# volume-em/empanada

Hardware: AMD Instinct MI355X
Metric: Mvox/s end-to-end 3D panoptic inference (incl. consensus); PQ vs CPU ref (higher is better)
Workload: dtype f32

## Files before the change

empanada_amd/_hip.py:

```python
import ctypes
import os

import torch

_HERE = os.path.dirname(os.path.abspath(__file__))
LIB_PATH = os.path.join(_HERE, 'libemp_hip.so')

MAX_KS = 11
MAX_CLASSES = 16
MAX_CENTERS = 4096


class HipError(RuntimeError):
    pass


_c = ctypes
_P = _c.c_void_p
_I = _c.c_int
_L = _c.c_int64
_F = _c.c_float
_U32 = _c.c_uint32

SIGNATURES = {
    'emp_version': (_I, []),
    'emp_last_error': (_c.c_char_p, []),
    'emp_device_count': (_I, []),
    'emp_bn_act_nhwc': (_I, [_P, _P, _P, _P, _I, _L, _I, _P, _L, _P]),
    'emp_dwconv_nhwc': (_I, [_P, _P, _P, _I, _I, _I, _I, _I, _P, _P]),
    'emp_upsample_bilinear': (_I, [_P, _I, _I, _I, _I, _P, _P, _I, _I, _P, _P]),
    'emp_conv_bn_act_proj_nhwc': (_I, [_P, _P, _P, _P, _I] + [_I] * 10 + [_P, _I, _P, _P, _L, _P]),
    'emp_conv_k_slab': (_I, [_L, _I, _I, _I]),
    'emp_conv_k_slab_cin': (_I, [_L, _I, _I, _I, _I]),
    'emp_conv_k_slab_geom': (_I, [_L, _I, _I, _I, _I, _I, _I, _I, _I]),
    'emp_conv1x1_ws_eligible': (_I, [_L, _I, _I, _I, _I, _I, _I, _I]),
    'emp_gconv_chunk': (_I, [_I]),
    'emp_gconv3x3_bn_act_nhwc': (_I, [_P, _L, _P, _P, _P, _I, _I, _I, _I, _I, _I, _I, _P, _L, _P]),
    'emp_conv_bn_act_nhwc': (_I, [_P, _P, _P, _P, _P, _L, _I] + [_I] * 10 + [_P, _L, _P]),
    'emp_conv_splitk_plan': (_I, [_L, _I, _I, _I, _I]),
    'emp_conv_splitk_bn_act_nhwc': (_I, [_P, _P, _P, _P, _P, _L, _I] + [_I] * 11 + [_P, _P, _L, _P]),
    'emp_wino_input_transform': (_I, [_P, _I, _I, _I, _I, _I, _P, _L, _P, _P]),
    'emp_gemm_nt_batched': (_I, [_P, _P, _I, _L, _I, _I, _P, _P]),
    'emp_wino4_input_transform': (_I, [_P, _I, _I, _I, _I, _I, _P, _L, _P, _P]),
    'emp_wino4_output_transform': (_I, [_P, _P, _L, _I, _I, _I, _I, _I, _P, _P, _I, _P, _L, _P]),
    'emp_wino3_input_transform': (_I, [_P, _I, _I, _I, _I, _I, _P, _L, _P, _P]),
    'emp_wino3_output_transform': (_I, [_P, _P, _L, _I, _I, _I, _I, _I, _P, _P, _I, _P, _L, _P]),
    'emp_wino_gemm_fused': (_I, [_P, _I, _I, _I, _I, _I, _P, _L, _P, _I, _P, _P]),
    'emp_wino_output_transform': (_I, [_P, _P, _L, _I, _I, _I, _I, _I, _P, _P, _I, _P, _L, _P]),
    'emp_chain_class': (_I, [_L, _P, _P, _P, _I, _P, _P, _P, _P, _L, _L, _c.c_double, _c.c_double, _P, _P, _P, _P]),
    'emp_lsap_maximize': (_L, [_P, _L, _L, _P, _P]),
    'emp_slices_to_input': (_I, [_P, _L, _L, _L, _I, _I, _I, _I, _I, _F, _F, _P, _P]),
    'emp_pointwise_out_nhwc': (_I, [_P, _P, _P, _L, _L, _I, _I, _P, _P]),
    'emp_bn_relu_maxpool_nhwc': (_I, [_P, _P, _P, _I, _I, _I, _I, _P, _P]),
    'emp_stem_conv7_bn_relu_maxpool': (_I, [_P, _P, _P, _P, _I, _I, _I, _P, _P]),
    'emp_logits_to_prob': (_I, [_P, _I, _I, _L, _P, _P]),
    'emp_pr_upsample2x': (_I, [_P, _I, _I, _I, _I, _P, _P, _P]),
    'emp_pr_topk_work_bytes': (_L, [_I, _L]),
    'emp_pr_topk': (_I, [_P, _I, _L, _I, _P, _L, _P, _P]),
    'emp_pr_point_sample': (_I, [_P, _L, _P, _I, _I, _I, _I, _I, _P, _I, _I, _I, _P, _P, _I, _P]),
    'emp_pr_scatter': (_I, [_P, _I, _P, _I, _I, _I, _L, _P, _P]),
    'emp_median_harden_stack': (_I, [_P, _I, _I, _L, _I, _F, _P, _P, _P]),
    'emp_median_step': (_I, [_c.POINTER(_P), _I, _L, _P, _P]),
    'emp_harden': (_I, [_P, _I, _I, _L, _F, _P, _P]),
    'emp_find_centers': (_I, [_P, _I, _I, _I, _F, _I, _I, _P, _P, _P]),
    'emp_group_work_elems': (_L, [_I, _I]),
    'emp_group_pixels': (_I, [_P, _P, _I, _P, _I, _I, _I, _I, _P, _U32, _P, _P, _P]),
    'emp_fuse_work_elems': (_L, [_I, _I, _I]),
    'emp_fuse_panoptic': (_I, [_P, _P, _I, _I, _I, _I, _I, _I, _U32, _L, _L, _L, _P, _P, _P, _P]),
    'emp_fuse_lut': (_I, [_P, _P, _I, _I, _I, _I, _I, _I, _U32, _L, _L, _P, _P]),
    'emp_fuse_apply': (_I, [_P, _P, _I, _I, _I, _I, _I, _I, _U32, _L, _L, _P, _P, _P, _P]),
    'emp_runs_count': (_I, [_P, _I, _I, _I, _P, _P]),
    'emp_scan_tmp_elems': (_L, [_L]),
    'emp_exclusive_scan_i32': (_I, [_P, _L, _P, _P, _P]),
    'emp_runs_extract': (_I, [_P, _I, _I, _I, _P, _P, _P, _P, _P]),
    'emp_runs_label_work_elems': (_L, [_L]),
    'emp_runs_label': (_I, [_P, _P, _P, _P, _L, _I, _I, _I, _L, _U32, _P, _P, _P, _P, _P, _P, _P, _P, _P]),
    'emp_runs_overlap_next': (_I, [_P, _P, _P, _P, _P, _L, _I, _I, _I, _L, _P, _L, _P, _P]),
    'emp_rle_decode': (_I, [_P, _P, _P, _L, _P, _P]),
    'emp_rle_encode_work_elems': (_L, [_L]),
    'emp_rle_encode': (_I, [_P, _L, _P, _P, _P, _P, _P]),
    'emp_box_pairs': (_I, [_P, _L, _P, _L, _I, _P, _P, _I, _P, _L, _P, _P]),
    'emp_rle_pair_intersections': (_I, [_P, _P, _P, _P, _L, _P, _P]),
    'emp_sort_work_bytes': (_L, [_L]),
    'emp_sort_u64_i32': (_I, [_P, _P, _P, _P, _L, _I, _I, _P, _L, _P]),
# ... 30 lines not shown
            fn = getattr(lib, name)
            fn.restype = res
            fn.argtypes = args
        _lib = lib
    return _lib


def require_gpu():
    if torch.cuda._is_in_bad_fork():
        raise HipError("this process was forked from one that had initialised the GPU: HIP cannot be used here.  Start "
                       "the process with the 'spawn' method (multiprocessing.set_start_method('spawn')), or call "
                       "patterns.forward_matching / forward_multigpu, which re-start themselves that way")
    if not torch.cuda.is_available():
        raise HipError("empanada_amd needs an MI355X (HIP device) for this operation; no CPU fallback exists")


def _ptr(t):
    if t is None:
        return None
    assert t.is_cuda and t.is_contiguous(), "device-resident contiguous tensor required"
    return t.data_ptr()


def as_u32(t):
    if t.dtype == torch.uint32:
        return t
    if t.dtype != torch.int32:
        t = t.to(torch.int32)
    return t.contiguous().view(torch.uint32)


def np_to_dev_u32(a):
    import numpy as np
    a = np.ascontiguousarray(a).astype(np.uint32)
    return torch.from_numpy(a.view(np.int32)).cuda().view(torch.uint32)


def stream():
    return torch.cuda.current_stream().cuda_stream


PROFILE = None
PROFILE_SKIP = set()
_TRACE = None
if os.environ.get('EMP_TRACE_CALLS'):
    _TRACE = open(os.environ['EMP_TRACE_CALLS'], 'a', buffering=1)


def trace(msg):
    if _TRACE is not None:
        _TRACE.write('# ' + msg + '\n')


def call(name, *args, alg_bytes=None, alg_flops=None):
    lib = load()
    if _TRACE is not None:
        _TRACE.write(name + ' ' + ' '.join(str(a) for a in args if isinstance(a, (int, float)) and abs(a) < (1 << 40))
                     + '\n')
    if PROFILE is not None and name not in PROFILE_SKIP:
        e0 = torch.cuda.Event(enable_timing=True)
        e1 = torch.cuda.Event(enable_timing=True)
        e0.record()
        rc = getattr(lib, name)(*args)
        e1.record()
        PROFILE.setdefault(name, []).append((e0, e1, alg_bytes, alg_flops))
    else:
        rc = getattr(lib, name)(*args)
    if rc != 0:
        raise HipError(f"{name} failed ({rc}): {lib.emp_last_error().decode()}")


def query(name, *args):
    return getattr(load(), name)(*args)


def median_harden_stack(prob, ks, thr, want_prob=False):
    require_gpu()
    D, C, H, W = prob.shape
    prob = prob.contiguous()
    sem = torch.empty((D, H, W), dtype=torch.uint8, device=prob.device)
    outp = torch.empty_like(prob) if want_prob else None
    call('emp_median_harden_stack', _ptr(prob), D, C, H * W, int(ks), float(thr), _ptr(sem), _ptr(outp), stream())
    return (sem, outp) if want_prob else sem


def _expect(what, t, dtype=None, shape=None, numel=None):
    if not isinstance(t, torch.Tensor) or not t.is_cuda:
        raise HipError(f"{what}: expected a tensor on the GPU")
    if dtype is not None and t.dtype not in (dtype if isinstance(dtype, tuple) else (dtype,)):
        raise HipError(f"{what}: dtype {t.dtype}, expected {dtype}")
    if shape is not None and tuple(t.shape) != tuple(shape):
        raise HipError(f"{what}: shape {tuple(t.shape)}, expected {tuple(shape)}")
    if numel is not None and t.numel() != numel:
        raise HipError(f"{what}: {t.numel()} elements, expected {numel}")
    return t


def median_step(slices, out=None):
    require_gpu()
    ks = len(slices)
    if not 1 <= ks <= MAX_KS:
        raise HipError(f"median over {ks} slices (1..{MAX_KS} supported)")
    for i, s in enumerate(slices):
        _expect(f"median_step: slice {i}", s, torch.float32, slices[0].shape)
    slices = [s.contiguous() for s in slices]
    n = slices[0].numel()
    if out is None:
        out = torch.empty_like(slices[0])
    _expect("median_step: out", out, torch.float32, numel=n)
    arr = (_P * ks)(*[s.data_ptr() for s in slices])
    call('emp_median_step', arr, ks, n, _ptr(out), stream())
    return out


def find_centers(hmp, thr, k, cap=1024):
    require_gpu()
    _expect("find_centers: heat map", hmp, torch.float32)
    D, h, w = hmp.shape
# ... 649 lines not shown
    g = w_oihw.detach().double().cpu()

    def comb(a, b, c):
        return [(G[0] * a + G[1] * b) + G[2] * c for G in _WINO3_G]

    rows = comb(g[:, :, 0, :], g[:, :, 1, :], g[:, :, 2, :])
    U = []
    for r in rows:
        U.extend(comb(r[:, :, 0], r[:, :, 1], r[:, :, 2]))
    return torch.stack(U, dim=0).float().contiguous()


def wino3_conv_bn_act(x, U, tiles_dev, dil, scale=None, shift=None, relu=False, out=None):
    require_gpu()
    N, Cin, H, W = x.shape
    Cout = U.shape[1]
    assert x.is_cuda and x.dtype == torch.float32 and x.is_contiguous(memory_format=torch.channels_last)
    T = tiles_dev.shape[0]
    V = torch.empty((25, T, Cin), dtype=torch.float32, device=x.device)
    Mw = torch.empty((25, T, Cout), dtype=torch.float32, device=x.device)
    if out is None:
        out = torch.empty((N, Cout, H, W), dtype=torch.float32, device=x.device, memory_format=torch.channels_last)
    assert out.shape == (N, Cout, H, W) and out.stride(1) == 1
    ops = out.stride(3)
    assert out.stride(2) == W * ops and out.stride(0) == H * W * ops, "NHWC channel slice required"
    st = stream()
    call('emp_wino3_input_transform', x.data_ptr(), N, H, W, Cin, dil, _ptr(tiles_dev), T, _ptr(V), st,
         alg_bytes=4 * (x.numel() + V.numel()))
    call('emp_gemm_nt_batched', _ptr(V), _ptr(U), 25, T, Cout, Cin, _ptr(Mw), st,
         alg_bytes=4 * (V.numel() + U.numel() + Mw.numel()), alg_flops=2 * 25 * T * Cout * Cin)
    call('emp_wino3_output_transform', _ptr(Mw), _ptr(tiles_dev), T, N, H, W, Cout, dil, _ptr(scale), _ptr(shift),
         int(bool(relu)), out.data_ptr(), ops, st, alg_bytes=4 * (Mw.numel() + N * Cout * H * W))
    return out


def conv_bn_act_proj_nhwc(x, w_okkc, scale, shift, relu, proj_w, proj_b=None, stride=1, pad=0, dil=1, keep=False):
    require_gpu()
    N, Cin, H, W = x.shape
    Cout, KH, KW, _ = w_okkc.shape
    n = proj_w.shape[0]
    assert x.is_cuda and x.dtype == torch.float32 and x.is_contiguous(memory_format=torch.channels_last)
    OH = (H + 2 * pad - dil * (KH - 1) - 1) // stride + 1
    OW = (W + 2 * pad - dil * (KW - 1) - 1) // stride + 1
    acc = torch.zeros((N, n, OH, OW), dtype=torch.float32, device=x.device)
    act = (torch.empty((N, Cout, OH, OW), dtype=torch.float32, device=x.device, memory_format=torch.channels_last)
           if keep else None)
    call('emp_conv_bn_act_proj_nhwc', x.data_ptr(), _ptr(w_okkc), _ptr(scale), _ptr(shift), int(bool(relu)), N, H, W,
         Cin, Cout, KH, KW, stride, pad, dil, _ptr(proj_w), n, _ptr(acc), act.data_ptr() if keep else None, 0,
         stream(), alg_bytes=4 * (x.numel() + w_okkc.numel() + acc.numel() + (act.numel() if keep else 0)),
         alg_flops=2 * N * OH * OW * Cout * (Cin * KH * KW + n))
    if proj_b is not None:
        acc += proj_b.view(1, -1, 1, 1)
    return (acc, act) if keep else acc
```

empanada_amd/csrc/emp_conv.hip:

```cpp
#include "emp_common.h"
#include <stdlib.h>

typedef float f32x16 __attribute__((ext_vector_type(16)));

#define CG_BM 128
#define CG_BK 32
#define CG_THREADS 256

struct ConvGeom {
    const float *x, *w, *scale, *shift, *res;
    float *out;
    int N, H, W, Cin, OH, OW, Cout, KH, KW, stride, pad, dil, relu;
    int64_t M, out_ps, res_ps;
    int tiles_m, tiles_n;
    int64_t x_bs, w_bs, out_bs;
    const int32_t *tiles;
    const float *proj_w;
    float *proj_out;
    int proj_n;
    int64_t hw;
};

__device__ __attribute__((aligned(16))) float cg_zero_page[64];

// ... 645 lines not shown
    const int T = g.tiles_m * g.tiles_n;
    const dim3 grid(8 * ((T + 7) / 8), 1, k_splits);
    hipStream_t st = emp_stream(stream);
    if (pl.narrow)
        hipLaunchKernelGGL((conv_igemm_f32_kernel<1, 0, false, 32, false, true>), grid, dim3(CG_THREADS), 0, st, g);
    else
        hipLaunchKernelGGL((conv_igemm_f32_kernel<2, 0, false, 32, false, true>), grid, dim3(CG_THREADS), 0, st, g);
    EMP_CHECK_LAUNCH("emp_conv_splitk_bn_act_nhwc(partials)");
    const int64_t total = g.M * (Cout / 4);
    hipLaunchKernelGGL(splitk_reduce_kernel, dim3(emp_grid(total, 256, 4096)), dim3(256), 0, st, work, k_splits, g.M, Cout,
                       scale, shift, residual, res_pixel_stride, relu, out, out_pixel_stride);
    EMP_CHECK_LAUNCH("emp_conv_splitk_bn_act_nhwc(reduce)");
    return EMP_OK;
}

extern "C" int emp_conv_bn_act_proj_nhwc(const float *x, const float *w_okkc, const float *scale, const float *shift,
                                         int relu, int N, int H, int W, int Cin, int Cout, int KH, int KW, int stride,
                                         int pad, int dil, const float *proj_w, int proj_n, float *proj_out,
                                         float *out, int64_t out_pixel_stride, void *stream)
{
    EMP_REQUIRE(x && w_okkc && proj_w && proj_out, "conv_proj: null pointer");
    EMP_REQUIRE(N >= 0 && H > 0 && W > 0 && Cin > 0 && Cin % CG_BK == 0, "conv_proj: bad shape (Cin %% %d)", CG_BK);
    EMP_REQUIRE(Cout == 128 || Cout == 256, "conv_proj: Cout %d must be 128 or 256 (at most two cout tiles)", Cout);
    EMP_REQUIRE(proj_n >= 1 && proj_n <= 4, "conv_proj: proj_n %d not in 1..4", proj_n);
    EMP_REQUIRE(KH >= 1 && KW >= 1 && KH <= 7 && KW <= 7 && stride >= 1 && dil >= 1 && pad >= 0, "conv_proj: bad filter geometry");
    const int OH = (H + 2 * pad - dil * (KH - 1) - 1) / stride + 1;
    const int OW = (W + 2 * pad - dil * (KW - 1) - 1) / stride + 1;
    EMP_REQUIRE(OH > 0 && OW > 0, "conv_proj: empty output");
    if (out_pixel_stride == 0) out_pixel_stride = Cout;
    EMP_REQUIRE(((reinterpret_cast<uintptr_t>(x) | reinterpret_cast<uintptr_t>(w_okkc) | reinterpret_cast<uintptr_t>(proj_w) |
                  reinterpret_cast<uintptr_t>(out)) & 15) == 0 && (out_pixel_stride & 3) == 0, "conv_proj: alignment");
    EMP_REQUIRE(out != x, "conv_proj: output cannot alias the input");
    if (N == 0) return EMP_OK;
    ConvGeom g;
    g.x = x; g.w = w_okkc; g.scale = scale; g.shift = shift; g.res = nullptr; g.out = out;
    g.N = N; g.H = H; g.W = W; g.Cin = Cin; g.OH = OH; g.OW = OW; g.Cout = Cout; g.KH = KH; g.KW = KW;
    g.stride = stride; g.pad = pad; g.dil = dil; g.relu = relu;
    g.M = (int64_t)N * OH * OW; g.out_ps = out_pixel_stride; g.res_ps = Cout;
    g.x_bs = g.w_bs = g.out_bs = 0; g.tiles = nullptr;
    g.proj_w = proj_w; g.proj_out = proj_out; g.proj_n = proj_n; g.hw = (int64_t)OH * OW;
    const CgPlan pl = cg_plan(g.M, Cout, 1, false, true, false);
    g.tiles_m = pl.tiles_m;
    g.tiles_n = pl.tiles_n;
    const int T = g.tiles_m * g.tiles_n;
    const int grid = 8 * ((T + 7) / 8);
#define CG_GOP(BK_, GL_) hipLaunchKernelGGL((conv_igemm_f32_kernel<2, 0, false, BK_, true, GL_>), dim3(grid), dim3(CG_THREADS), 0, emp_stream(stream), g)
    if (pl.glds) { if (pl.slab == 16) CG_GOP(16, true); else CG_GOP(32, true); }
    else { if (pl.slab == 16) CG_GOP(16, false); else CG_GOP(32, false); }
#undef CG_GOP
    EMP_CHECK_LAUNCH("emp_conv_bn_act_proj_nhwc");
    return EMP_OK;
}


__global__ __launch_bounds__(256) void wino_input_kernel(const float *__restrict__ x, const int32_t *__restrict__ tiles,
                                                         int64_t T, int H, int W, int C4, int dil, float4 *__restrict__ V)
{
    const int64_t total = T * C4;
    for (int64_t i = (int64_t)blockIdx.x * blockDim.x + threadIdx.x; i < total; i += (int64_t)gridDim.x * blockDim.x) {
        const int c4 = (int)(i % C4);
        const int64_t t = i / C4;
        const int n = tiles[3 * t], by = tiles[3 * t + 1], bx = tiles[3 * t + 2];
        const float4 *src = reinterpret_cast<const float4 *>(x) + (int64_t)n * H * W * C4 + c4;
        float4 d[4][4];
#pragma unroll
        for (int a = 0; a < 4; ++a)
#pragma unroll
            for (int b = 0; b < 4; ++b) {
                const int yy = by + a * dil, xx = bx + b * dil;
                d[a][b] = make_float4(0.f, 0.f, 0.f, 0.f);
                if (yy >= 0 && yy < H && xx >= 0 && xx < W) d[a][b] = src[((int64_t)yy * W + xx) * C4];
            }
#define W_SUB(p, q) make_float4(__fsub_rn(p.x, q.x), __fsub_rn(p.y, q.y), __fsub_rn(p.z, q.z), __fsub_rn(p.w, q.w))
#define W_ADD(p, q) make_float4(__fadd_rn(p.x, q.x), __fadd_rn(p.y, q.y), __fadd_rn(p.z, q.z), __fadd_rn(p.w, q.w))
        float4 tt[4][4];
#pragma unroll
        for (int a = 0; a < 4; ++a) {
            tt[a][0] = W_SUB(d[a][0], d[a][2]);
            tt[a][1] = W_ADD(d[a][1], d[a][2]);
            tt[a][2] = W_SUB(d[a][2], d[a][1]);
            tt[a][3] = W_SUB(d[a][1], d[a][3]);
        }
        float4 *dst = V + t * C4 + c4;
        const int64_t ps = T * C4;
#pragma unroll
        for (int v = 0; v < 4; ++v) {
            dst[(0 * 4 + v) * ps] = W_SUB(tt[0][v], tt[2][v]);
            dst[(1 * 4 + v) * ps] = W_ADD(tt[1][v], tt[2][v]);
            dst[(2 * 4 + v) * ps] = W_SUB(tt[2][v], tt[1][v]);
            dst[(3 * 4 + v) * ps] = W_SUB(tt[1][v], tt[3][v]);
        }
    }
}

__global__ __launch_bounds__(256) void wino_output_kernel(const float4 *__restrict__ Mw, const int32_t *__restrict__ tiles,
                                                          int64_t T, int H, int W, int Co4, int dil,
                                                          const float4 *__restrict__ scale, const float4 *__restrict__ shift,
                                                          int relu, float *__restrict__ out, int64_t out_ps)
{
    const int64_t total = T * Co4;
    for (int64_t i = (int64_t)blockIdx.x * blockDim.x + threadIdx.x; i < total; i += (int64_t)gridDim.x * blockDim.x) {
        const int c4 = (int)(i % Co4);
        const int64_t t = i / Co4;
        const int n = tiles[3 * t], oy = tiles[3 * t + 1] + dil, ox = tiles[3 * t + 2] + dil;
        const float4 *src = Mw + t * Co4 + c4;
        const int64_t ps = T * Co4;
// ... 409 lines not shown
```

empanada_amd/models/panoptic_deeplab.py:

```python
import zlib
from typing import List

import torch
import torch.nn as nn
import torch.nn.functional as F

__all__ = ['PanopticDeepLab', 'PanopticDeepLabPR', 'PointRendSemSegHead', 'resnet_encoder', 'prepare_for_inference',
           'tune_fused_convs',
           'synthesize_weights']

_RESNETS = {
    'resnet18': ('basic', [2, 2, 2, 2]), 'resnet34': ('basic', [3, 4, 6, 3]),
    'resnet50': ('bottleneck', [3, 4, 6, 3]), 'resnet101': ('bottleneck', [3, 4, 23, 3]),
    'resnet152': ('bottleneck', [3, 8, 36, 3]),
}


def _conv_bn_act(nin, nout, k, stride=1, groups=1, act=True):
    layers = [nn.Conv2d(nin, nout, k, stride=stride, padding=(k - 1) // 2, groups=groups, bias=False),
              nn.BatchNorm2d(nout)]
    if act:
        layers.append(nn.ReLU(inplace=True))
    return nn.Sequential(*layers)


class SeparableConv2d(nn.Module):

    def __init__(self, nin, nout, kernel_size=3, stride=1, bias=True):
        super().__init__()
        self.sepconv = nn.Sequential(
            nn.Conv2d(nin, nin, kernel_size, stride=stride, padding=(kernel_size - 1) // 2, groups=nin, bias=bias),
            nn.Conv2d(nin, nout, 1, stride=1, bias=bias))

    def forward(self, x):
        return self.sepconv(x)


def _sepconv_bn_act(nin, nout, k):
    return nn.Sequential(SeparableConv2d(nin, nout, k, 1, bias=False), nn.BatchNorm2d(nout), nn.ReLU(inplace=True))


def _bn_affine(bn):
    scale = (bn.weight.detach().float() / torch.sqrt(bn.running_var.detach().float() + bn.eps)).contiguous()
    shift = (bn.bias.detach().float() - bn.running_mean.detach().float() * scale).contiguous()
    return scale, shift


def _no_late_weights(state_dict, prefix, *args):
    raise RuntimeError("load_state_dict after prepare_for_inference: load the weights into the plain model first "
                       f"(module {prefix.rstrip('.')!r} holds folded copies)")


class DepthwiseConvNHWC(nn.Module):

    def __init__(self, conv):
        super().__init__()
        k = conv.kernel_size[0]
        C = conv.in_channels
        self.register_buffer('w_kkc', conv.weight.detach().float().reshape(C, k * k).t().contiguous())
        self.register_buffer('b', conv.bias.detach().float().contiguous() if conv.bias is not None else None)
        self.k = k

    @staticmethod
    def eligible(m):
        return (isinstance(m, nn.Conv2d) and m.groups == m.in_channels == m.out_channels and m.in_channels % 4 == 0
                and m.kernel_size[0] == m.kernel_size[1] and m.kernel_size[0] in (3, 5) and m.stride == (1, 1)
                and m.dilation == (1, 1) and m.padding == (m.kernel_size[0] // 2,) * 2
                and m.padding_mode == 'zeros')

    def forward(self, x):
        from .. import _hip
        if not x.is_contiguous(memory_format=torch.channels_last):
            x = x.contiguous(memory_format=torch.channels_last)
        return _hip.dwconv_nhwc(x, self.w_kkc, self.b, self.k)


class FusedBNAct(nn.Module):

    def __init__(self, bn, relu):
        super().__init__()
        scale, shift = _bn_affine(bn)
        self.register_buffer('scale', scale, persistent=False)
        self.register_buffer('shift', shift, persistent=False)
        self.relu = relu
        self._register_load_state_dict_pre_hook(_no_late_weights)

    def forward(self, x, residual=None, out=None):
        from .. import _hip
# ... 331 lines not shown
        return self.project(torch.cat([conv(x) for conv in self.convs], dim=1))


class PanopticDeepLabDecoder(nn.Module):

    def __init__(self, in_channels, decoder_channels, low_level_stages, low_level_channels,
                 low_level_channels_project, atrous_rates, aspp_channels=None, aspp_dropout=0.5):
        super().__init__()
        aspp_channels = aspp_channels or decoder_channels
        self.aspp = ASPP(in_channels, aspp_channels, atrous_rates, aspp_dropout)
        self.low_level_stages = list(low_level_stages)
        project, fuse = [], []
        for i, (lc, pc) in enumerate(zip(low_level_channels, low_level_channels_project)):
            project.append(_conv_bn_act(lc, pc, 1))
            fuse.append(_sepconv_bn_act((aspp_channels if i == 0 else decoder_channels) + pc, decoder_channels, 5))
        self.project = nn.ModuleList(project)
        self.fuse = nn.ModuleList(fuse)
        self.hip_ops = False

    def forward(self, pyramid: List[torch.Tensor]):
        x = self.aspp(pyramid[-1])
        for stage, proj, fuse in zip(self.low_level_stages, self.project, self.fuse):
            feat = pyramid[stage]
            if self.hip_ops and _can_write_into(proj, feat):
                cx = x.shape[1]
                cl = (proj[0].conv if isinstance(proj[0], FusedConvBNAct) else proj[0]).out_channels
                buf = torch.empty((x.shape[0], cx + cl, feat.shape[2], feat.shape[3]), dtype=x.dtype,
                                  device=x.device, memory_format=torch.channels_last)
                _up_bilinear(x, feat.shape[2:], True, out=buf[:, :cx])
                _conv_bn_into(proj, feat, buf[:, cx:])
                x = fuse(buf)
            else:
                low = proj(feat)
                x = _up_bilinear(x, low.shape[2:], self.hip_ops)
                x = fuse(torch.cat((x, low), dim=1))
        return x


class PanopticDeepLabHead(nn.Module):

    def __init__(self, nin, n_classes):
        super().__init__()
        self.head = nn.Sequential(_sepconv_bn_act(nin, nin, 5), nn.Conv2d(nin, n_classes, 1, bias=True))
        self.hip_ops = False

    def forward(self, x):
        if self.hip_ops and x.is_cuda and x.dtype == torch.float32:
            sep = self.head[0][0]
            site = sep.sepconv[1] if isinstance(sep, SeparableConv2d) else None
            last = self.head[1]
            if (isinstance(site, FusedConvBNAct) and site.impl == 'direct' and isinstance(last, PointwiseOutNHWC)
                    and site.conv.out_channels in (128, 256) and site.conv.kernel_size == (1, 1)):
                from .. import _hip
                y = sep.sepconv[0](x)
                if not y.is_contiguous(memory_format=torch.channels_last):
                    y = y.contiguous(memory_format=torch.channels_last)
                site._prepare('direct')
                return _hip.conv_bn_act_proj_nhwc(y, site._w_okkc, site.bn.scale, site.bn.shift, site.bn.relu,
                                                  last.w, last.b)
        return self.head(x)


class PanopticDeepLab(nn.Module):

    def __init__(self, encoder='resnet50', num_classes=1, stage4_stride=16, decoder_channels=256,
                 low_level_stages=(3, 2, 1), low_level_channels_project=(128, 64, 32), atrous_rates=(2, 4, 6),
                 aspp_channels=None, aspp_dropout=0.1, ins_decoder=False, ins_ratio=0.5, **kwargs):
        super().__init__()
        assert encoder in _RESNETS, f'Invalid encoder name {encoder}, choices are {sorted(_RESNETS)}'
        assert stage4_stride in (16, 32) and min(low_level_stages) > 0
        self.decoder_channels = decoder_channels
        self.num_classes = num_classes
        self.encoder = resnet_encoder(encoder, output_stride=stage4_stride)
        sem_p, ins_p = (aspp_dropout, aspp_dropout) if isinstance(aspp_dropout, float) else aspp_dropout
        widths = self.encoder.cfg.widths
        low_ch = [int(widths[i - 1]) for i in low_level_stages]
        self.semantic_decoder = PanopticDeepLabDecoder(int(widths[-1]), decoder_channels, low_level_stages, low_ch,
                                                       list(low_level_channels_project), atrous_rates,
                                                       aspp_channels, sem_p)
        if ins_decoder:
            self.instance_decoder = PanopticDeepLabDecoder(
                int(widths[-1]), decoder_channels, low_level_stages, low_ch,
                [int(s * ins_ratio) for s in low_level_channels_project], atrous_rates, aspp_channels, ins_p)
        else:
            self.instance_decoder = None
        self.semantic_head = PanopticDeepLabHead(decoder_channels, num_classes)
        self.ins_center = PanopticDeepLabHead(decoder_channels, 1)
        self.ins_xy = PanopticDeepLabHead(decoder_channels, 2)

    hip_ops = False

    def _up4(self, x):
        return _up_bilinear(x, (4 * x.shape[2], 4 * x.shape[3]), self.hip_ops)

    def forward(self, x):
        pyramid = self.encoder(x)
        sem_x = self.semantic_decoder(pyramid)
        ins_x = sem_x if self.instance_decoder is None else self.instance_decoder(pyramid)
        return {'sem_logits': self._up4(self.semantic_head(sem_x)),
                'ctr_hmp': self._up4(self.ins_center(ins_x)),
                'offsets': self._up4(self.ins_xy(ins_x))}


class StandardPointHead(nn.Module):

    def __init__(self, nin, num_classes, fc_dim, num_fc):
# ... 250 lines not shown
```

include/emp_hip.h:

```cpp
#ifndef EMP_HIP_H
#define EMP_HIP_H

#include <stdint.h>

#ifdef __cplusplus
extern "C" {
#endif

#define EMP_OK 0
#define EMP_EINVAL (-1)
#define EMP_ELAUNCH (-2)
#define EMP_ENODEV (-3)

#define EMP_MAX_KS 11
#define EMP_MAX_CLASSES 16
#define EMP_MAX_CENTERS 4096

int emp_version(void);
const char *emp_last_error(void);
int emp_device_count(void);

int emp_slices_to_input(const uint8_t *vol, int64_t stride_slice, int64_t stride_row, int64_t stride_col,
                        int n_slices, int h, int w, int hp, int wp, float mean255, float inv_std255,
                        float *out, void *stream);

int emp_bn_act_nhwc(const float *x, const float *scale, const float *shift, const float *residual,
                    int relu, int64_t n_pixels, int C, float *out, int64_t out_pixel_stride, void *stream);

int emp_dwconv_nhwc(const float *x, const float *w_kkc, const float *bias, int N, int H, int W, int C,
                    int k, float *y, void *stream);

int emp_upsample_bilinear(const float *x, int N, int C, int h, int w, const int64_t *x_strides,
                          float *y, int H, int W, const int64_t *y_strides, void *stream);

int emp_conv_k_slab(int64_t M, int Cout, int batch, int has_residual);
int emp_conv_k_slab_cin(int64_t M, int Cout, int batch, int has_residual, int Cin);
int emp_conv_k_slab_geom(int64_t M, int Cout, int has_residual, int Cin, int KH, int KW, int stride, int pad, int relu);
int emp_conv1x1_ws_eligible(int64_t M, int Cin, int Cout, int KH, int KW, int stride, int pad, int relu);
int emp_conv_bn_act_nhwc(const float *x, const float *w_okkc, const float *scale, const float *shift,
                         const float *residual, int64_t res_pixel_stride, int relu, int N, int H, int W,
                         int Cin, int Cout, int KH, int KW, int stride, int pad, int dil, float *out,
                         int64_t out_pixel_stride, void *stream);
int emp_conv_splitk_plan(int64_t M, int Cout, int Cin, int KH, int KW);
int emp_conv_splitk_bn_act_nhwc(const float *x, const float *w_okkc, const float *scale, const float *shift,
                                const float *residual, int64_t res_pixel_stride, int relu, int N, int H, int W,
                                int Cin, int Cout, int KH, int KW, int stride, int pad, int dil, int k_splits,
                                float *work, float *out, int64_t out_pixel_stride, void *stream);

int emp_conv_bn_act_proj_nhwc(const float *x, const float *w_okkc, const float *scale, const float *shift,
                              int relu, int N, int H, int W, int Cin, int Cout, int KH, int KW, int stride,
                              int pad, int dil, const float *proj_w, int proj_n, float *proj_out,
                              float *out, int64_t out_pixel_stride, void *stream);

int emp_gconv_chunk(int group_w);
int emp_gconv3x3_bn_act_nhwc(const float *x, int64_t x_pixel_stride, const float *w_okkc, const float *scale,
                             const float *shift, int relu, int N, int H, int W, int groups, int group_w,
                             int stride, float *out, int64_t out_pixel_stride, void *stream);

int emp_wino_input_transform(const float *x, int N, int H, int W, int C, int dil, const int32_t *tiles,
                             int64_t T, float *V, void *stream);
int emp_gemm_nt_batched(const float *A, const float *B, int batch, int64_t M, int N, int K, float *C,
                        void *stream);
int emp_wino_gemm_fused(const float *x, int N, int H, int W, int Cin, int dil, const int32_t *tiles,
                        int64_t T, const float *U, int Cout, float *Mw, void *stream);
int emp_wino_output_transform(const float *Mw, const int32_t *tiles, int64_t T, int N, int H, int W,
                              int Cout, int dil, const float *scale, const float *shift, int relu,
                              float *out, int64_t out_pixel_stride, void *stream);

int emp_wino4_input_transform(const float *x, int N, int H, int W, int C, int dil, const int32_t *tiles,
                              int64_t T, float *V, void *stream);
int emp_wino4_output_transform(const float *Mw, const int32_t *tiles, int64_t T, int N, int H, int W,
                               int Cout, int dil, const float *scale, const float *shift, int relu,
                               float *out, int64_t out_pixel_stride, void *stream);

int emp_wino3_input_transform(const float *x, int N, int H, int W, int C, int dil, const int32_t *tiles,
                              int64_t T, float *V, void *stream);
int emp_wino3_output_transform(const float *Mw, const int32_t *tiles, int64_t T, int N, int H, int W,
                               int Cout, int dil, const float *scale, const float *shift, int relu,
                               float *out, int64_t out_pixel_stride, void *stream);

int emp_pointwise_out_nhwc(const float *x, const float *w, const float *bias, int64_t n_pixels,
                           int64_t pixels_per_image, int C, int Cout, float *out, void *stream);

int emp_bn_relu_maxpool_nhwc(const float *x, const float *scale, const float *shift, int N, int H, int W,
                             int C, float *y, void *stream);

int emp_stem_conv7_bn_relu_maxpool(const float *x, const float *w_tc, const float *scale, const float *shift,
                                   int N, int H, int W, float *y, void *stream);

int emp_logits_to_prob(const float *logits, int N, int C, int64_t HW, float *prob, void *stream);

int emp_median_harden_stack(const float *prob, int D, int C, int64_t HW, int ks, float thr,
                            uint8_t *out_sem, float *out_prob, void *stream);

int emp_median_step(const float *const *slices_host, int ks, int64_t n, float *out, void *stream);

int emp_harden(const float *prob, int D, int C, int64_t HW, float thr, uint8_t *out_sem,
               void *stream);

int emp_find_centers(const float *hmp, int D, int h, int w, float thr, int k, int cap,
                     int32_t *out_idx, int32_t *out_count, void *stream);

int64_t emp_group_work_elems(int D, int cap);
int emp_group_pixels(const int32_t *ctr_idx, const int32_t *ctr_count, int cap,
                     const float *offsets, int D, int h, int w, int step, const uint8_t *sem,
// ... 115 lines not shown
```

Baseline: 127.9.

## Fuse 5x5 depthwise conv into pointwise implicit-GEMM conv kernel

Adds a new HIP kernel that computes the 5x5 depthwise convolution on an input halo patch staged in LDS, writes the result straight into the A tile, and then runs the 1x1 pointwise conv with BN/ReLU (and an optional projection head) using MFMA. The separable-conv blocks in the DeepLab decoder and heads take this path by default when the geometry check passes. This removes the round trip of the depthwise intermediate through global memory and one kernel launch per block. In exchange the depthwise work is recomputed over halo regions, LDS use per block rises, and occupancy may fall.

```diff
diff --git a/empanada_amd/_hip.py b/empanada_amd/_hip.py
--- a/empanada_amd/_hip.py
+++ b/empanada_amd/_hip.py
@@ -30,6 +30,10 @@
     'emp_dwconv_nhwc': (_I, [_P, _P, _P, _I, _I, _I, _I, _I, _P, _P]),
     'emp_upsample_bilinear': (_I, [_P, _I, _I, _I, _I, _P, _P, _I, _I, _P, _P]),
     'emp_conv_bn_act_proj_nhwc': (_I, [_P, _P, _P, _P, _I] + [_I] * 10 + [_P, _I, _P, _P, _L, _P]),
+    'emp_dwconv_conv_fused_ok': (_I, [_I] * 8),
+    'emp_dwconv_conv_bn_act_nhwc': (_I, [_P, _P, _P, _I, _P, _P, _P, _I, _I, _I, _I, _I, _I, _P, _L, _P]),
+    'emp_dwconv_conv_bn_act_proj_nhwc': (_I, [_P, _P, _P, _I, _P, _P, _P, _I, _I, _I, _I, _I, _I, _P, _I, _P, _P, _L,
+                                              _P]),
     'emp_conv_k_slab': (_I, [_L, _I, _I, _I]),
     'emp_conv_k_slab_cin': (_I, [_L, _I, _I, _I, _I]),
     'emp_conv_k_slab_geom': (_I, [_L, _I, _I, _I, _I, _I, _I, _I, _I]),
@@ -166,18 +170,19 @@
         _TRACE.write('# ' + msg + '\n')
 
 
-def call(name, *args, alg_bytes=None, alg_flops=None):
+def call(name, *args, alg_bytes=None, alg_flops=None, profile_as=None):
     lib = load()
     if _TRACE is not None:
         _TRACE.write(name + ' ' + ' '.join(str(a) for a in args if isinstance(a, (int, float)) and abs(a) < (1 << 40))
                      + '\n')
-    if PROFILE is not None and name not in PROFILE_SKIP:
+    pname = profile_as or name
+    if PROFILE is not None and pname not in PROFILE_SKIP:
         e0 = torch.cuda.Event(enable_timing=True)
         e1 = torch.cuda.Event(enable_timing=True)
         e0.record()
         rc = getattr(lib, name)(*args)
         e1.record()
-        PROFILE.setdefault(name, []).append((e0, e1, alg_bytes, alg_flops))
+        PROFILE.setdefault(pname, []).append((e0, e1, alg_bytes, alg_flops))
     else:
         rc = getattr(lib, name)(*args)
     if rc != 0:
@@ -933,3 +938,55 @@
     if proj_b is not None:
         acc += proj_b.view(1, -1, 1, 1)
     return (acc, act) if keep else acc
+
+
+SEPCONV_FUSED = os.environ.get('EMP_SEPCONV_FUSED', '1') != '0'
+
+
+def dwconv_conv_fused_ok(x, w_kkc, k, w_oc, relu, proj=False):
+    N, Cin, H, W = x.shape
+    Cout = w_oc.shape[0]
+    if w_oc.dim() != 4 or tuple(w_oc.shape[1:]) != (1, 1, Cin) or tuple(w_kkc.shape) != (k * k, Cin):
+        return False
+    return bool(load().emp_dwconv_conv_fused_ok(N, H, W, Cin, Cout, int(k), int(bool(relu)), int(bool(proj))))
+
+
+def _sep_operands(name, x, w_kkc, bias, k, w_oc, scale, shift):
+    require_gpu()
+    N, Cin, H, W = x.shape
+    Cout = w_oc.shape[0]
+    assert x.is_cuda and x.dtype == torch.float32 and x.is_contiguous(memory_format=torch.channels_last)
+    _expect(f"{name}: depthwise weights", w_kkc, torch.float32, (k * k, Cin))
+    _expect(f"{name}: pointwise weights", w_oc, torch.float32, (Cout, 1, 1, Cin))
+    for what, t, n in (("bias", bias, Cin), ("scale", scale, Cout), ("shift", shift, Cout)):
+        if t is not None:
+            _expect(f"{name}: {what}", t, torch.float32, (n,))
+    return N, Cin, H, W, Cout
+
+
+def dwconv_conv_bn_act_nhwc(x, w_kkc, bias, k, w_oc, scale=None, shift=None, relu=False, out=None):
+    N, Cin, H, W, Cout = _sep_operands("dwconv_conv", x, w_kkc, bias, k, w_oc, scale, shift)
+    if out is None:
+        out = torch.empty((N, Cout, H, W), dtype=torch.float32, device=x.device, memory_format=torch.channels_last)
+    assert out.shape == (N, Cout, H, W) and out.dtype == torch.float32 and out.stride(1) == 1
+    ops = out.stride(3)
+    assert out.stride(2) == W * ops and out.stride(0) == H * W * ops, "NHWC channel slice required"
+    call('emp_dwconv_conv_bn_act_nhwc', x.data_ptr(), _ptr(w_kkc), _ptr(bias), int(k), _ptr(w_oc), _ptr(scale),
+         _ptr(shift), int(bool(relu)), N, H, W, Cin, Cout, out.data_ptr(), ops, stream(),
+         alg_bytes=4 * (x.numel() + w_kkc.numel() + w_oc.numel() + N * Cout * H * W),
+         alg_flops=2 * N * H * W * Cout * Cin, profile_as='emp_conv_bn_act_nhwc')
+    return out
+
+
+def dwconv_conv_bn_act_proj_nhwc(x, w_kkc, bias, k, w_oc, scale, shift, relu, proj_w, proj_b=None):
+    N, Cin, H, W, Cout = _sep_operands("dwconv_conv_proj", x, w_kkc, bias, k, w_oc, scale, shift)
+    n = proj_w.shape[0]
+    _expect("dwconv_conv_proj: proj weights", proj_w, torch.float32, (n, Cout))
+    acc = torch.zeros((N, n, H, W), dtype=torch.float32, device=x.device)
+    call('emp_dwconv_conv_bn_act_proj_nhwc', x.data_ptr(), _ptr(w_kkc), _ptr(bias), int(k), _ptr(w_oc), _ptr(scale),
+         _ptr(shift), int(bool(relu)), N, H, W, Cin, Cout, _ptr(proj_w), n, _ptr(acc), None, 0, stream(),
+         alg_bytes=4 * (x.numel() + w_kkc.numel() + w_oc.numel() + acc.numel()),
+         alg_flops=2 * N * H * W * Cout * (Cin + n), profile_as='emp_conv_bn_act_proj_nhwc')
+    if proj_b is not None:
+        acc += proj_b.view(1, -1, 1, 1)
+    return acc
diff --git a/empanada_amd/csrc/emp_conv.hip b/empanada_amd/csrc/emp_conv.hip
--- a/empanada_amd/csrc/emp_conv.hip
+++ b/empanada_amd/csrc/emp_conv.hip
@@ -721,6 +721,323 @@
     return EMP_OK;
 }
 
+#define SC_PH 8
+#define SC_PW 16
+#define SC_K 5
+
+struct SepGeom {
+    const float *x, *wdw, *bias, *w, *scale, *shift;
+    float *out;
+    const float *proj_w;
+    float *proj_out;
+    int N, H, W, Cin, Cout, relu, proj_n;
+    int tiles_x, tiles_y, T;
+    int64_t out_ps;
+};
+
+template <int NT, int BK, bool PROJ>
+__global__ __launch_bounds__(CG_THREADS, (BK == 16 ? 2 : 1)) void sepconv_igemm_f32_kernel(SepGeom g)
+{
+    constexpr int P = SC_K / 2;
+    constexpr int BN = 64 * NT;
+    constexpr int CPP = BK / 4;
+    constexpr int HW = SC_PW + SC_K - 1, HP = (SC_PH + SC_K - 1) * HW;
+    constexpr int WD0 = HP * CPP;
+    constexpr int B0 = WD0 + (SC_K * SC_K + 1) * CPP;
+    constexpr int NCH = B0 + BN * CPP;
+    constexpr int SLOT = (NCH + 63) / 64 * 64;
+    constexpr int NR = (SLOT + CG_THREADS - 1) / CG_THREADS;
+    constexpr int A_OFF = 2 * SLOT * 4;
+    constexpr int NF4 = BK / 8;
+    constexpr int CLD = BN + 4;
+    constexpr int EPI_ROWS = 64;
+    constexpr int LOOP_F = A_OFF + CG_BM * BK;
+    constexpr int SMEM = LOOP_F > EPI_ROWS * CLD ? LOOP_F : EPI_ROWS * CLD;
+    constexpr int NB = CG_THREADS / (CPP * SC_PW);
+    constexpr int RY = SC_PH / NB;
+    static_assert(SC_PH * SC_PW == CG_BM && NB * RY == SC_PH, "patch / tile mismatch");
+    __shared__ __attribute__((aligned(16))) float smem[SMEM];
+
+    const int chunk = (g.T + 7) >> 3;
+    const int tile = (blockIdx.x & 7) * chunk + (blockIdx.x >> 3);
+    if (tile >= g.T) return;
+    const int tx = tile % g.tiles_x, ty = (tile / g.tiles_x) % g.tiles_y, n = tile / (g.tiles_x * g.tiles_y);
+    const int y0 = ty * SC_PH, x0 = tx * SC_PW;
+    const int tid = threadIdx.x, wave = tid >> 6, lane = tid & 63;
+
+    const float *src[NR];
+    unsigned adv = 0;
+#pragma unroll
+    for (int k = 0; k < NR; ++k) {
+        const int idx = k * CG_THREADS + tid;
+        const float *s = cg_zero_page;
+        bool ok = false;
+        if (idx < WD0) {
+            const int h = idx / CPP, q = idx % CPP;
+            const int iy = y0 - P + h / HW, ix = x0 - P + h % HW;
+            if (iy >= 0 && iy < g.H && ix >= 0 && ix < g.W) {
+                s = g.x + (((int64_t)n * g.H + iy) * g.W + ix) * g.Cin + 4 * q;
+                ok = true;
+            }
+        } else if (idx < B0) {
+            const int t = (idx - WD0) / CPP, q = (idx - WD0) % CPP;
+            if (t < SC_K * SC_K) {
+                s = g.wdw + (int64_t)t * g.Cin + 4 * q;
+                ok = true;
+            } else if (g.bias) {
+                s = g.bias + 4 * q;
+                ok = true;
+            }
+        } else if (idx < NCH) {
+            const int row = (idx - B0) / CPP, pq = (idx - B0) % CPP;
+            const int swz = (BK == 16) ? ((row >> 2) & 3) : ((row >> 1) & 7);
+            s = g.w + (int64_t)row * g.Cin + 4 * (pq ^ swz);
+            ok = true;
+        }
+        src[k] = s;
+        adv |= ok ? (1u << k) : 0u;
+    }
+    const unsigned lds0 = (unsigned)(size_t)(__attribute__((address_space(3))) float *)smem;
+    const unsigned dst0 = __builtin_amdgcn_readfirstlane(lds0 + (unsigned)(wave * 64 * 16));
+    auto issue = [&](int slot, int c0) {
+#pragma unroll
+        for (int k = 0; k < NR; ++k)
+            if (k * CG_THREADS + wave * 64 < SLOT)
+                cg_glds16(src[k] + (((adv >> k) & 1u) ? c0 : 0), dst0 + (unsigned)((slot * SLOT + k * CG_THREADS) * 16));
+    };
+
+    float *As = smem + A_OFF;
+    const int dq = tid % CPP, dpx = (tid / CPP) % SC_PW, band = tid / (CPP * SC_PW);
+    auto depthwise = [&](int slot) {
+        const float4 *Hs = reinterpret_cast<const float4 *>(smem) + slot * SLOT;
+        float4 a[RY];
+#pragma unroll
+        for (int k = 0; k < RY; ++k) a[k] = make_float4(0.f, 0.f, 0.f, 0.f);
+#pragma unroll 1
+        for (int rr = 0; rr < RY + SC_K - 1; ++rr) {
+            float4 in[SC_K];
+#pragma unroll
+            for (int j = 0; j < SC_K; ++j) in[j] = Hs[((band * RY + rr) * HW + dpx + j) * CPP + dq];
+#pragma unroll
+            for (int k = 0; k < RY; ++k) {
+                const int i = rr - k;
+                if (i < 0 || i >= SC_K) continue;
+#pragma unroll
+                for (int j = 0; j < SC_K; ++j) {
+                    const float4 wv = Hs[WD0 + (i * SC_K + j) * CPP + dq];
+                    a[k].x = fmaf(in[j].x, wv.x, a[k].x);
+                    a[k].y = fmaf(in[j].y, wv.y, a[k].y);
+                    a[k].z = fmaf(in[j].z, wv.z, a[k].z);
+                    a[k].w = fmaf(in[j].w, wv.w, a[k].w);
+                }
+            }
+        }
+        const float4 b = Hs[WD0 + SC_K * SC_K * CPP + dq];
+#pragma unroll
+        for (int k = 0; k < RY; ++k) {
+            const int m = (band * RY + k) * SC_PW + dpx;
+            const int swz = (BK == 16) ? ((m >> 2) & 3) : ((m >> 1) & 7);
+            *reinterpret_cast<float4 *>(As + m * BK + 4 * (dq ^ swz)) =
+                make_float4(__fadd_rn(a[k].x, b.x), __fadd_rn(a[k].y, b.y), __fadd_rn(a[k].z, b.z), __fadd_rn(a[k].w, b.w));
+        }
+    };
+
+    const int wm = wave >> 1, wn = wave & 1;
+    const int r = lane & 31, hh = lane >> 5;
+    f32x16 acc[2][NT];
+#pragma unroll
+    for (int i = 0; i < 2; ++i)
+#pragma unroll
+        for (int j = 0; j < NT; ++j)
+#pragma unroll
+            for (int q = 0; q < 16; ++q) acc[i][j][q] = 0.f;
+
+    const int S = g.Cin / BK;
+    const int swz_rd = (BK == 16) ? ((r >> 2) & 3) : ((r >> 1) & 7);
+    issue(0, 0);
+    cg_wait_vm<0>();
+    __syncthreads();
+    for (int s = 0; s < S; ++s) {
+        const int slot = s & 1;
+        if (s + 1 < S) issue(slot ^ 1, (s + 1) * BK);
+        depthwise(slot);
+        __syncthreads();
+        const float *Ar = As + (wm * 64 + r) * BK;
+        const float *Br = smem + (slot * SLOT + B0) * 4 + (wn * 32 * NT + r) * BK;
+#pragma unroll
+        for (int f = 0; f < NF4; ++f) {
+            const int pc = (((hh * NF4 + f) ^ swz_rd) * 4);
+            float4 fa[2], fb[NT];
+#pragma unroll
+            for (int i = 0; i < 2; ++i) fa[i] = *reinterpret_cast<const float4 *>(Ar + i * 32 * BK + pc);
+#pragma unroll
+            for (int j = 0; j < NT; ++j) fb[j] = *reinterpret_cast<const float4 *>(Br + j * 32 * BK + pc);
+#pragma unroll
+            for (int e = 0; e < 4; ++e) {
+                float av[2], bv[NT];
+#pragma unroll
+                for (int i = 0; i < 2; ++i) av[i] = e == 0 ? fa[i].x : e == 1 ? fa[i].y : e == 2 ? fa[i].z : fa[i].w;
+#pragma unroll
+                for (int j = 0; j < NT; ++j) bv[j] = e == 0 ? fb[j].x : e == 1 ? fb[j].y : e == 2 ? fb[j].z : fb[j].w;
+#pragma unroll
+                for (int i = 0; i < 2; ++i)
+#pragma unroll
+                    for (int j = 0; j < NT; ++j)
+                        acc[i][j] = __builtin_amdgcn_mfma_f32_32x32x2f32(av[i], bv[j], acc[i][j], 0, 0, 0);
+            }
+        }
+        cg_wait_vm<0>();
+        __syncthreads();
+    }
+
+    constexpr int C4 = BN / 4, RPI = CG_THREADS / C4, NRR = EPI_ROWS / RPI;
+    float *Cs = smem;
+    const int ccol = (tid % C4) * 4, crow = tid / C4;
+    float sc[4] = {1.f, 1.f, 1.f, 1.f}, sh[4] = {0.f, 0.f, 0.f, 0.f};
+#pragma unroll
+    for (int e = 0; e < 4; ++e) {
+        if (g.scale) sc[e] = g.scale[ccol + e];
+        if (g.shift) sh[e] = g.shift[ccol + e];
+    }
+#pragma unroll
+    for (int rd = 0; rd < 2; ++rd) {
+        if (rd > 0) __syncthreads();
+        if (wm == rd) {
+#pragma unroll
+            for (int i = 0; i < 2; ++i)
+#pragma unroll
+                for (int j = 0; j < NT; ++j)
+#pragma unroll
+                    for (int q = 0; q < 16; ++q)
+                        Cs[(i * 32 + (q & 3) + 8 * (q >> 2) + 4 * hh) * CLD + wn * 32 * NT + j * 32 + r] = acc[i][j][q];
+        }
+        __syncthreads();
+#pragma unroll
+        for (int it = 0; it < NRR; ++it) {
+            const int lrow_c = crow + it * RPI;
+            const int m = rd * EPI_ROWS + lrow_c;
+            const int y = y0 + m / SC_PW, xx = x0 + m % SC_PW;
+            const bool valid = y < g.H && xx < g.W;
+            const int64_t p = ((int64_t)n * g.H + y) * g.W + xx;
+            float v[4] = {0.f, 0.f, 0.f, 0.f};
+            if (valid) {
+                const float4 a4 = *reinterpret_cast<const float4 *>(&Cs[lrow_c * CLD + ccol]);
+                v[0] = a4.x; v[1] = a4.y; v[2] = a4.z; v[3] = a4.w;
+#pragma unroll
+                for (int e = 0; e < 4; ++e) {
+                    if (g.scale) v[e] = __fmul_rn(v[e], sc[e]);
+                    if (g.shift) v[e] = __fadd_rn(v[e], sh[e]);
+                    if (g.relu) v[e] = fmaxf(v[e], 0.f);
+                }
+                if (!PROJ || g.out)
+                    *reinterpret_cast<float4 *>(g.out + p * g.out_ps + ccol) = make_float4(v[0], v[1], v[2], v[3]);
+            }
+            if constexpr (PROJ) {
+                float ps[4] = {0.f, 0.f, 0.f, 0.f};
+                if (valid) {
+#pragma unroll
+                    for (int q = 0; q < 4; ++q)
+                        if (q < g.proj_n) {
+                            const float4 wq = *reinterpret_cast<const float4 *>(g.proj_w + (int64_t)q * g.Cout + ccol);
+                            ps[q] = __fadd_rn(__fadd_rn(__fadd_rn(__fmul_rn(v[0], wq.x), __fmul_rn(v[1], wq.y)),
+                                                        __fmul_rn(v[2], wq.z)), __fmul_rn(v[3], wq.w));
+                        }
+                }
+                *reinterpret_cast<float4 *>(&Cs[lrow_c * CLD + ccol]) = make_float4(ps[0], ps[1], ps[2], ps[3]);
+            }
+        }
+        if constexpr (PROJ) {
+            constexpr int HALVES = BN / 128;
+            __syncthreads();
+            for (int idx = tid; idx < EPI_ROWS * g.proj_n * HALVES; idx += CG_THREADS) {
+                const int row_l = idx / (g.proj_n * HALVES), rem = idx - row_l * (g.proj_n * HALVES);
+                const int q = rem / HALVES, hf = rem - q * HALVES;
+                const int m = rd * EPI_ROWS + row_l;
+                const int y = y0 + m / SC_PW, xx = x0 + m % SC_PW;
+                if (y < g.H && xx < g.W) {
+                    const float *c = Cs + row_l * CLD + hf * 128 + q;
+                    float t = c[0];
+#pragma unroll 8
+                    for (int j = 1; j < 32; ++j) t = __fadd_rn(t, c[4 * j]);
+                    atomicAdd(g.proj_out + ((int64_t)n * g.proj_n + q) * ((int64_t)g.H * g.W) + (int64_t)y * g.W + xx, t);
+                }
+            }
+        }
+    }
+}
+
+extern "C" int emp_dwconv_conv_fused_ok(int N, int H, int W, int Cin, int Cout, int k, int relu, int proj)
+{
+    if (N < 1 || H < 1 || W < 1 || k != SC_K || (Cout != 128 && Cout != 256) || Cin < 32 || relu < 0 || relu > 1) return 0;
+    if (Cin % (proj ? 32 : 16) != 0) return 0;
+    const int64_t T = (int64_t)N * emp_cdiv(H, SC_PH) * emp_cdiv(W, SC_PW);
+    if (T >= (1LL << 28)) return 0;
+    if (!proj && emp_conv1x1_ws_eligible((int64_t)N * H * W, Cin, Cout, 1, 1, 1, 0, relu)) return 0;
+    return 1;
+}
+
+static int sepconv_launch(const char *name, const float *x, const float *w_kkc, const float *bias, int k,
+                          const float *w_oc, const float *scale, const float *shift, int relu, int N, int H, int W,
+                          int Cin, int Cout, const float *proj_w, int proj_n, float *proj_out, float *out,
+                          int64_t out_pixel_stride, void *stream)
+{
+    const bool proj = proj_w != nullptr;
+    EMP_REQUIRE(x && w_kkc && w_oc && (proj ? proj_out != nullptr : out != nullptr), "%s: null pointer", name);
+    EMP_REQUIRE(N >= 0 && H > 0 && W > 0, "%s: bad shape", name);
+    EMP_REQUIRE(!proj || (proj_n >= 1 && proj_n <= 4), "%s: proj_n %d not in 1..4", name, proj_n);
+    EMP_REQUIRE(N == 0 || emp_dwconv_conv_fused_ok(N, H, W, Cin, Cout, k, relu, proj),
+                "%s: geometry not covered (k %d, Cin %d, Cout %d, relu %d): see emp_dwconv_conv_fused_ok", name, k,
+                Cin, Cout, relu);
+    if (out_pixel_stride == 0) out_pixel_stride = Cout;
+    EMP_REQUIRE(out_pixel_stride >= Cout && (out_pixel_stride & 3) == 0, "%s: bad pixel stride", name);
+    EMP_REQUIRE(((reinterpret_cast<uintptr_t>(x) | reinterpret_cast<uintptr_t>(w_kkc) | reinterpret_cast<uintptr_t>(bias) |
+                  reinterpret_cast<uintptr_t>(w_oc) | reinterpret_cast<uintptr_t>(scale) | reinterpret_cast<uintptr_t>(shift) |
+                  reinterpret_cast<uintptr_t>(proj_w) | reinterpret_cast<uintptr_t>(out)) & 15) == 0,
+                "%s: pointers must be 16-byte aligned", name);
+    EMP_REQUIRE(out != x, "%s: output cannot alias the input", name);
+    if (N == 0) return EMP_OK;
+    SepGeom g;
+    g.x = x; g.wdw = w_kkc; g.bias = bias; g.w = w_oc; g.scale = scale; g.shift = shift; g.out = out;
+    g.proj_w = proj_w; g.proj_out = proj_out; g.proj_n = proj ? proj_n : 0;
+    g.N = N; g.H = H; g.W = W; g.Cin = Cin; g.Cout = Cout; g.relu = relu; g.out_ps = out_pixel_stride;
+    g.tiles_x = (int)emp_cdiv(W, SC_PW);
+    g.tiles_y = (int)emp_cdiv(H, SC_PH);
+    g.T = N * g.tiles_x * g.tiles_y;
+    const int64_t M = (int64_t)N * H * W;
+    const int slab = proj ? cg_plan(M, Cout, 1, false, true, false).slab : cg_plan(M, Cout, 1, false, true, true, Cin).slab;
+    const int grid = 8 * ((g.T + 7) / 8);
+#define SC_GO(NT_, BK_, PR_) hipLaunchKernelGGL((sepconv_igemm_f32_kernel<NT_, BK_, PR_>), dim3(grid), dim3(CG_THREADS), 0, emp_stream(stream), g)
+    if (Cout == 256) {
+        if (slab == 16) { if (proj) SC_GO(4, 16, true); else SC_GO(4, 16, false); }
+        else { if (proj) SC_GO(4, 32, true); else SC_GO(4, 32, false); }
+    } else {
+        if (slab == 16) { if (proj) SC_GO(2, 16, true); else SC_GO(2, 16, false); }
+        else { if (proj) SC_GO(2, 32, true); else SC_GO(2, 32, false); }
+    }
+#undef SC_GO
+    EMP_CHECK_LAUNCH(name);
+    return EMP_OK;
+}
+
+extern "C" int emp_dwconv_conv_bn_act_nhwc(const float *x, const float *w_kkc, const float *bias, int k,
+                                           const float *w_oc, const float *scale, const float *shift, int relu, int N,
+                                           int H, int W, int Cin, int Cout, float *out, int64_t out_pixel_stride,
+                                           void *stream)
+{
+    return sepconv_launch("dwconv_conv", x, w_kkc, bias, k, w_oc, scale, shift, relu, N, H, W, Cin, Cout, nullptr, 0,
+                          nullptr, out, out_pixel_stride, stream);
+}
+
+extern "C" int emp_dwconv_conv_bn_act_proj_nhwc(const float *x, const float *w_kkc, const float *bias, int k,
+                                                const float *w_oc, const float *scale, const float *shift, int relu,
+                                                int N, int H, int W, int Cin, int Cout, const float *proj_w, int proj_n,
+                                                float *proj_out, float *out, int64_t out_pixel_stride, void *stream)
+{
+    EMP_REQUIRE(proj_w, "dwconv_conv_proj: null pointer");
+    return sepconv_launch("dwconv_conv_proj", x, w_kkc, bias, k, w_oc, scale, shift, relu, N, H, W, Cin, Cout, proj_w,
+                          proj_n, proj_out, out, out_pixel_stride, stream);
+}
+
 
 __global__ __launch_bounds__(256) void wino_input_kernel(const float *__restrict__ x, const int32_t *__restrict__ tiles,
                                                          int64_t T, int H, int W, int C4, int dil, float4 *__restrict__ V)
diff --git a/empanada_amd/models/panoptic_deeplab.py b/empanada_amd/models/panoptic_deeplab.py
--- a/empanada_amd/models/panoptic_deeplab.py
+++ b/empanada_amd/models/panoptic_deeplab.py
@@ -33,7 +33,31 @@
             nn.Conv2d(nin, nout, 1, stride=1, bias=bias))
 
     def forward(self, x):
+        site = self.fused_site(x)
+        if site is not None:
+            from .. import _hip
+            dw = self.sepconv[0]
+            if not x.is_contiguous(memory_format=torch.channels_last):
+                x = x.contiguous(memory_format=torch.channels_last)
+            return _hip.dwconv_conv_bn_act_nhwc(x, dw.w_kkc, dw.b, dw.k, site._w_okkc, site.bn.scale, site.bn.shift,
+                                                site.bn.relu)
         return self.sepconv(x)
+
+    def fused_site(self, x, proj=False):
+        dw, site = self.sepconv[0], self.sepconv[1]
+        if not (isinstance(dw, DepthwiseConvNHWC) and isinstance(site, FusedConvBNAct) and site.impl == 'direct'
+                and x.is_cuda and x.dtype == torch.float32):
+            return None
+        from .. import _hip
+        c = site.conv
+        if (not _hip.SEPCONV_FUSED or c.kernel_size != (1, 1) or c.stride != (1, 1) or c.padding != (0, 0)
+                or c.dilation != (1, 1) or c.groups != 1 or c.bias is not None):
+            return None
+        site._prepare('direct')
+        if not _hip.dwconv_conv_fused_ok(x, dw.w_kkc, dw.k, site._w_okkc, site.bn.relu, proj):
+            return None
+        site._seen = (tuple(x.shape), False)
+        return site
 
 
 def _sepconv_bn_act(nin, nout, k):
@@ -471,6 +495,13 @@
             if (isinstance(site, FusedConvBNAct) and site.impl == 'direct' and isinstance(last, PointwiseOutNHWC)
                     and site.conv.out_channels in (128, 256) and site.conv.kernel_size == (1, 1)):
                 from .. import _hip
+                fsite = sep.fused_site(x, proj=True)
+                if fsite is not None:
+                    dw = sep.sepconv[0]
+                    if not x.is_contiguous(memory_format=torch.channels_last):
+                        x = x.contiguous(memory_format=torch.channels_last)
+                    return _hip.dwconv_conv_bn_act_proj_nhwc(x, dw.w_kkc, dw.b, dw.k, site._w_okkc, site.bn.scale,
+                                                             site.bn.shift, site.bn.relu, last.w, last.b)
                 y = sep.sepconv[0](x)
                 if not y.is_contiguous(memory_format=torch.channels_last):
                     y = y.contiguous(memory_format=torch.channels_last)
diff --git a/include/emp_hip.h b/include/emp_hip.h
--- a/include/emp_hip.h
+++ b/include/emp_hip.h
@@ -51,6 +51,15 @@
                               int relu, int N, int H, int W, int Cin, int Cout, int KH, int KW, int stride,
                               int pad, int dil, const float *proj_w, int proj_n, float *proj_out,
                               float *out, int64_t out_pixel_stride, void *stream);
+
+int emp_dwconv_conv_fused_ok(int N, int H, int W, int Cin, int Cout, int k, int relu, int proj);
+int emp_dwconv_conv_bn_act_nhwc(const float *x, const float *w_kkc, const float *bias, int k, const float *w_oc,
+                                const float *scale, const float *shift, int relu, int N, int H, int W, int Cin,
+                                int Cout, float *out, int64_t out_pixel_stride, void *stream);
+int emp_dwconv_conv_bn_act_proj_nhwc(const float *x, const float *w_kkc, const float *bias, int k, const float *w_oc,
+                                     const float *scale, const float *shift, int relu, int N, int H, int W, int Cin,
+                                     int Cout, const float *proj_w, int proj_n, float *proj_out, float *out,
+                                     int64_t out_pixel_stride, void *stream);
 
 int emp_gconv_chunk(int group_w);
 int emp_gconv3x3_bn_act_nhwc(const float *x, int64_t x_pixel_stride, const float *w_okkc, const float *scale,
```

Result: no change. 129.1 (median of 6 runs) (+0.9%).
